# ha7ilm/csdr

Measured on AMD Instinct MI355X. Metric: complex MS/s in->out, WFM demod chain @2.4 MS/s x N streams, higher is better.
Workload: dtype f32

## Files before the change

### csdr_amd/csrc/wfm.hip

```cpp
#include "common.hpp"
#include "wfm_mfma.hpp"
#include "seeds.hpp"
#include <math.h>
#include <stdlib.h>
#include <vector>
#include <string>
#include <string.h>
using namespace csdr_amd;

namespace {

constexpr int HIST = WFM_HIST;
constexpr int TILE_A = 64;
constexpr int WARM = 48;

struct WfmParams {
    int D, L, F;
    int T;
    long long B;
    long long j_first;
    int n_audio;
};

__device__ __forceinline__ float u8_to_f(uint32_t v) { return fmaf((float)v, 0x1.010102p-7f, -1.0f); }
// ... 140 lines not shown
    size_t max_block;
    DevBuf<float> d_taps, d_demod, d_last[2];
    float phase;
    DevBuf<cf32> d_rot;
    DevBuf<uint8_t> d_hist;
    DevBuf<uint8_t> d_head[2]; int hflip;
    size_t demod_pitch;
    long long B, next_j;
    int last_T, flip;
    bool ended;
    std::string kernel_name;
    bool profiling;
    KernelTimer timer;
    double prof_ms; long prof_launches;
    bool use_mfma;
    WfmMfmaDevice mfma;
    DevBuf<> seq_frags; DevBuf<float> seq_cum; DevBuf<float2> dtab;
    DevBuf<float2> d_ctab; size_t ctab_cap;
    float2 c_prev;
    long long tab_first; bool tab_valid;
    bool ps; std::vector<float> rates, h_taps; DevBuf<float> d_scales;
    DevBuf<float2> d_dtab_old; DevBuf<int> d_lead_n; int *d_list; DevBuf<float> d_lead_d; std::vector<int> retuned;
    Owned<csdr_amd::SeedTables, seeds_destroy> seeds;
};

extern "C" {

static int wfm_upload_stream_tables(csdr_amd_wfm *w, int s, float rate)
{
    WfmMfmaTable t;
    wfm_mfma_build_table(w->D, w->L, w->F, rate, w->h_taps.data(), t);
    CSDR_HIP(hipMemcpy((uint8_t *)w->mfma.d_seq_frags + (size_t)s * t.seq_frags.size(), t.seq_frags.data(), t.seq_frags.size(), hipMemcpyHostToDevice));
    CSDR_HIP(hipMemcpy(w->mfma.d_seq_cum + (size_t)s * t.seq_cum.size(), t.seq_cum.data(), t.seq_cum.size() * sizeof(float), hipMemcpyHostToDevice));
    CSDR_HIP(hipMemcpy(w->mfma.d_dtab + (size_t)s * t.dtab.size(), t.dtab.data(), t.dtab.size() * sizeof(float2), hipMemcpyHostToDevice));
    CSDR_HIP(hipMemcpy(w->d_scales.get() + s, &t.seq_scale, sizeof(float), hipMemcpyHostToDevice));
    return 0;
}

static csdr_amd_wfm *wfm_create_impl(csdr_amd_ctx *ctx, int n_streams, const float *rates, bool per_stream, int decimation, const float *host_taps,
                                     int taps_length, int frac_rate, float tau, int audio_rate, size_t max_block_samples)
{
    const float shift_rate = rates ? rates[0] : 0.f;
    if (n_streams <= 0 || decimation <= 0 || taps_length <= 0 || frac_rate <= 1 || !rates) { fail_msg(-3, "wfm: bad parameters"); return nullptr; }
    if (decimation * 1 + taps_length + 8 > HIST) { fail_msg(-3, "wfm: D + taps (%d + %d) exceed the %d-sample history", decimation, taps_length, HIST); return nullptr; }
    if (max_block_samples < 1024) max_block_samples = 1024;
    Owned<csdr_amd_wfm, csdr_amd_wfm_destroy> w(new csdr_amd_wfm());
// ... 13 lines not shown
    alloc(w->d_taps, sizeof(float) * taps_length);
    alloc(w->d_last[0], sizeof(float) * n_streams);
    alloc(w->d_last[1], sizeof(float) * n_streams);
    if (w->use_mfma) {
        alloc(w->d_head[0], wfm_mfma_head_bytes(n_streams));
        alloc(w->d_head[1], wfm_mfma_head_bytes(n_streams));
    } else {
        alloc(w->d_demod, sizeof(float) * w->demod_pitch * n_streams);
        alloc(w->d_rot, sizeof(cf32) * (HIST + max_block_samples + 64));
        alloc(w->d_hist, (size_t)2 * HIST * n_streams);
    }
    if (e != hipSuccess) { fail(e, "hipMalloc(wfm state)", __FILE__, __LINE__); return nullptr; }
    (void)hipMemcpy(w->d_taps.get(), host_taps, sizeof(float) * taps_length, hipMemcpyHostToDevice);
    w->kernel_name = "k_wfm_front";
    if (w->use_mfma && per_stream) {
        WfmMfmaTable t;
        wfm_mfma_build_table(decimation, taps_length, frac_rate, shift_rate, host_taps, t);
        w->mfma.tile_stride_bytes = t.tile_stride_bytes; w->mfma.win_off_bytes = t.win_off_bytes; w->mfma.seq_scale = t.seq_scale;
        w->rates.assign(rates, rates + n_streams); w->h_taps.assign(host_taps, host_taps + taps_length);
        hipError_t e2 = dev_alloc(w->seq_frags, t.seq_frags.size() * (size_t)n_streams);
        if (e2 == hipSuccess) e2 = dev_alloc(w->seq_cum, t.seq_cum.size() * sizeof(float) * (size_t)n_streams);
        if (e2 == hipSuccess) e2 = dev_alloc(w->dtab, t.dtab.size() * sizeof(float2) * (size_t)n_streams);
        if (e2 == hipSuccess) e2 = dev_alloc(w->d_scales, sizeof(float) * (size_t)n_streams);
        w->mfma.d_seq_frags = w->seq_frags.get(); w->mfma.d_seq_cum = w->seq_cum.get(); w->mfma.d_dtab = w->dtab.get();
        if (e2 != hipSuccess) { fail(e2, "hipMalloc(wfm per-stream tables)", __FILE__, __LINE__); return nullptr; }
        for (int s = 0; s < n_streams; s++) if (wfm_upload_stream_tables(w.get(), s, rates[s])) return nullptr;
        w->seeds.reset(seeds_create(ctx, n_streams, rates, nullptr, 0, max_block_samples));
        if (!w->seeds) return nullptr;
        w->kernel_name = "k_wfm_mfma_seq";
    } else if (w->use_mfma) {
        WfmMfmaTable t;
        wfm_mfma_build_table(decimation, taps_length, frac_rate, shift_rate, host_taps, t);
        w->mfma.tile_stride_bytes = t.tile_stride_bytes; w->mfma.win_off_bytes = t.win_off_bytes; w->mfma.seq_scale = t.seq_scale;
        w->ctab_cap = 16 * (max_block_samples / 1024 + 8);
        hipError_t e2 = dev_alloc(w->d_ctab, w->ctab_cap * sizeof(float2));
        if (e2 == hipSuccess) e2 = dev_alloc(w->seq_frags, t.seq_frags.size());
        if (e2 == hipSuccess) e2 = dev_alloc(w->seq_cum, t.seq_cum.size() * sizeof(float));
        if (e2 == hipSuccess) e2 = dev_alloc(w->dtab, t.dtab.size() * sizeof(float2));
        w->mfma.d_seq_frags = w->seq_frags.get(); w->mfma.d_seq_cum = w->seq_cum.get(); w->mfma.d_dtab = w->dtab.get();
        if (e2 == hipSuccess) e2 = hipMemcpy(w->mfma.d_seq_frags, t.seq_frags.data(), t.seq_frags.size(), hipMemcpyHostToDevice);
        if (e2 == hipSuccess) e2 = hipMemcpy(w->mfma.d_seq_cum, t.seq_cum.data(), t.seq_cum.size() * sizeof(float), hipMemcpyHostToDevice);
        if (e2 == hipSuccess) e2 = hipMemcpy(w->mfma.d_dtab, t.dtab.data(), t.dtab.size() * sizeof(float2), hipMemcpyHostToDevice);
        if (e2 != hipSuccess) { fail(e2, "hipMalloc/hipMemcpy(wfm mfma table)", __FILE__, __LINE__); return nullptr; }
        w->kernel_name = "k_wfm_mfma_seq";
    }
    w->profiling = false; w->prof_ms = 0; w->prof_launches = 0;
// ... 126 lines not shown
    } else {
        if (w->last_T) CSDR_HIP(hipMemcpyAsync(w->d_rot.get(), w->d_rot.get() + w->last_T, sizeof(cf32) * HIST, hipMemcpyDeviceToDevice, st));
        rc = csdr_amd_rotator_generate(c, CSDR_SHIFT_ADDITION, w->shift_rate, &w->phase, w->d_rot.get() + HIST, (size_t)T, 1024, 0);
        if (rc) return rc;
    }
    const long long avail_last = w->B + T - 1;
    long long j_hi = -1;
    if (avail_last - (w->L - 1) >= 0) {
        const long long k_max = (avail_last - (w->L - 1)) / w->D;
        if (k_max >= 10) j_hi = (k_max - 10) / w->F;
    }
    const long long n_audio_ll = j_hi - w->next_j + 1;
    const int n_audio = n_audio_ll > 0 ? (int)n_audio_ll : 0;
    if (n_audio > 0 && (size_t)n_audio > out_pitch) return fail_msg(-3, "wfm: out_pitch %zu smaller than the %d audio samples of this block", out_pitch, n_audio);
    hipEvent_t e0 = nullptr, e1 = nullptr;
    if (w->profiling && n_audio > 0) { if (const int trc = w->timer.take(&e0, &e1)) return trc; }
    if (w->use_mfma) {
        WfmBackArgs back;
        back.alpha = w->alpha; back.last_in = w->d_last[w->flip].get(); back.last_out = w->d_last[w->flip ^ 1].get();
        back.s16 = audio_s16; back.af = audio_f; back.out_pitch = out_pitch; back.head_in = w->d_head[w->hflip].get(); back.head_out = w->d_head[w->hflip ^ 1].get();
        WfmPerStream psa; memset(&psa, 0, sizeof psa);
        if (w->ps) {
            psa.tab_pitch = sv.pitch; psa.tab_len = sv.n_entries; psa.d_scales = w->d_scales.get();
            long n_lead = 0; const int lead_max = wfm_lead_max(w->D, w->L, w->F);
            psa.lead_stride = lead_max;
            if (!w->retuned.empty() && n_audio > 0) {
                const long long lim = w->B - 1 - 9LL * w->D;
                if (lim >= 0) n_lead = (long)(lim / ((long long)w->D * w->F) - w->next_j + 1);
                if (n_lead < 0) n_lead = 0;
                if (n_lead > lead_max) n_lead = lead_max;
                if (n_lead > n_audio) n_lead = n_audio;
            }
            if (n_lead > 0) {
                const int nr = (int)w->retuned.size(), S = w->n_streams;
                if (!w->d_lead_n) { CSDR_HIP(dev_alloc(w->d_lead_n, sizeof(int) * 2 * S)); w->d_list = w->d_lead_n.get() + S; CSDR_HIP(dev_alloc(w->d_lead_d, sizeof(float) * (size_t)lead_max * S)); }
                int *hl = (int *)c->pinned_acquire(sizeof(int) * (size_t)(S + nr)); if (!hl) return -2;
                for (int s = 0; s < S; s++) hl[s] = 0;
                for (int k = 0; k < nr; k++) { hl[w->retuned[k]] = (int)n_lead; hl[S + k] = w->retuned[k]; }
                rc = c->pinned_upload(w->d_lead_n.get(), sizeof(int) * (size_t)(S + nr)); if (rc) return rc;
                rc = wfm_mfma_lead(st, in, in_pitch, back.head_in, w->d_taps.get(), sv.ctab, sv.pitch, w->mfma.d_dtab, w->d_dtab_old.get(), w->d_list, nr, w->d_lead_d.get(), lead_max,
                                   w->D, w->L, w->F, w->B, w->next_j, (int)n_lead);
                if (rc) return rc;
                psa.d_lead_d = w->d_lead_d.get(); psa.d_lead_n = w->d_lead_n.get();
            }
        }
        rc = wfm_mfma_launch(st, e0, e1, in, in_pitch, w->mfma, ctab_call, w->n_streams, T, w->B, w->next_j, n_audio, back, w->ps ? &psa : nullptr);
// ... 33 lines not shown
```

### csdr_amd/csrc/wfm_mfma.hip

```cpp
#include "common.hpp"
#include "wfm_mfma.hpp"
#include <hip/hip_ext.h>
#include <math.h>
#include <string.h>
#include <stdlib.h>
#include <complex>
#include <vector>
using namespace csdr_amd;

namespace csdr_amd {

bool wfm_mfma_supported(int D, int L, int F)
{
    if ((D * F) & 1) return false;
    const int win_off = (18 * D) & ~15;
    const int span_bytes = 2 * (D * (3 * F + 10) + L) - win_off;
    if (span_bytes > 64 * WFM_NK) return false;
    if (D + L + 3 * D * F + 8 > WFM_HIST) return false;
    return true;
}

void wfm_mfma_build_table(int D, int L, int F, float shift_rate, const float *taps, WfmMfmaTable &t)
{
    t.D = D; t.L = L; t.F = F;
// ... 89 lines not shown
#pragma unroll
            for (int l = 0; l < 3; l++) acc[l] = __builtin_amdgcn_mfma_i32_16x16x64_i8(A[ks * 3 + l], lo, acc[l], 0, 0, 0);
#pragma unroll
            for (int l = 0; l < 3; l++) snap[l] = acc[l];
#pragma unroll
            for (int l = 0; l < 3; l++) acc[l] = __builtin_amdgcn_mfma_i32_16x16x64_i8(A[ks * 3 + l], hi, acc[l], 0, 0, 0);
        } else {
#pragma unroll
            for (int l = 0; l < 3; l++) acc[l] = __builtin_amdgcn_mfma_i32_16x16x64_i8(A[ks * 3 + l], Bf[ks], acc[l], 0, 0, 0);
        }
    }
}

struct SeqParams {
    int n_streams; long long B2; long long tile_first; int n_tiles, tiles_per_seg;
    int stride, win_off; float scale;
    long long two_T;
    float alpha; const float *last_in; float *last_out; int16_t *s16; float *af; size_t out_pitch; long long j_first; int n_audio;
    const uint8_t *head_in; uint8_t *head_out;
    long long col_bytes; int col_chunks, col_audio, n_cols;
    size_t frag_stride, tab_pitch; int tab_len;
    const float *scales;
    const float *lead_d; const int *lead_n; int lead_stride;
};

#ifndef SEQ_RB_KIB
#define SEQ_RB_KIB 9
#endif
constexpr int SEQ_RB = 1024 * SEQ_RB_KIB;
#ifndef SEQ_RING_PAD
#define SEQ_RING_PAD 32
#endif
constexpr int SEQ_RP = SEQ_RB + SEQ_RING_PAD;
constexpr int SEQ_NGR = 4 * WFM_NK;
#ifndef SEQ_TPG_N
#define SEQ_TPG_N 6
#endif
#ifndef SEQ_NLD_N
#define SEQ_NLD_N 2
#endif
constexpr int SEQ_TPG = SEQ_TPG_N;
constexpr int SEQ_NLD = SEQ_NLD_N;
constexpr int SEQ_NW = SEQ_TPG + SEQ_NLD;
constexpr int SEQ_NLW = SEQ_NLD;
constexpr int SEQ_LINE = 64;
constexpr int SEQ_OUTS = (SEQ_LINE - 1 + 3 * 4 * SEQ_TPG + 4 * SEQ_TPG - 1) / (4 * SEQ_TPG);
// ... 14 lines not shown
#endif

constexpr int RES_WARM = 48;
struct ResCtl {
    const uint32_t *desc;
    const uint32_t *ctrl;
    uint32_t *done;
    unsigned *cnt;
    unsigned long long *t_first;
    unsigned long long *next_item;
    unsigned *exiting;
    const uint8_t *in_ring; int16_t *out_ring; size_t in_slot_bytes, out_slot_elems;
    int n_slots, desc_lines, n_wsb, T, D, L, F;
    long long idle_ticks, life_ticks;
    const float *lead_d; int lead_stride;
    const float *lead_state;
    unsigned long long *stats;
    int fence_mode;
};
__device__ __forceinline__ uint32_t sys_load(const uint32_t *p) { return __hip_atomic_load(p, __ATOMIC_RELAXED, __HIP_MEMORY_SCOPE_SYSTEM); }
__device__ __forceinline__ uint32_t res_tag(long long k) { return (uint32_t)((unsigned long long)k % 0xfffffffeull) + 1u; }

template <bool PS, bool RES = false>
__global__ __launch_bounds__(64 * SEQ_NW) void k_wfm_mfma_seq(const uint8_t *__restrict__ in, size_t in_pitch, const v4i *__restrict__ frags, const float *__restrict__ cum,
                                                               const float2 *__restrict__ dtab, const float2 *__restrict__ ctab, SeqParams p_in, ResCtl rc)
{
    static_assert(!(PS && RES), "the resident form exists for the shared-rate kernel");
    constexpr int TPG = SEQ_TPG, SPW = 16 / SEQ_NLW, NTHR = 64 * SEQ_NW;
    extern __shared__ float4 lds_raw[];
    uint8_t *lds_in = reinterpret_cast<uint8_t *>(lds_raw);
    float *lds_out = reinterpret_cast<float *>(lds_in + 16 * SEQ_RP);
    float *lcum = lds_out + 16 * SEQ_OUTP;
    float2 *ctl = reinterpret_cast<float2 *>(lcum + (SEQ_NGR + 1) * 16);
    const int tid = threadIdx.x, wv = __builtin_amdgcn_readfirstlane(tid >> 6), lane = tid & 63, col = lane & 15, q = lane >> 4;
    const bool fetches = wv >= TPG;
#ifdef WFM_PROF
    const long long t_entry = __builtin_readcyclecounter();
    long long t_first = t_entry, t_last = t_entry;
#endif
    const int fw = wv - TPG;
    float scale = p_in.scale;
    if constexpr (PS) { const int sbp = blockIdx.x; frags += (size_t)sbp * p_in.frag_stride; cum += (size_t)sbp * ((SEQ_NGR + 1) * 16); dtab += (size_t)sbp * 3072; ctab += sbp; scale = p_in.scales[sbp]; }
    for (int i = tid; i < (SEQ_NGR + 1) * 16; i += NTHR) lcum[i] = cum[i];
    v4i A[WFM_NK * 3];
#pragma unroll
    for (int s = 0; s < WFM_NK * 3; s++) A[s] = frags[s * 64 + lane];

    float c_lo[4], c_hi[4];
    {
        const float4 a = *reinterpret_cast<const float4 *>(cum + 4 * q), b = *reinterpret_cast<const float4 *>(cum + (size_t)SEQ_NGR * 16 + 4 * q);
        c_lo[0] = a.x; c_lo[1] = a.y; c_lo[2] = a.z; c_lo[3] = a.w; c_hi[0] = b.x; c_hi[1] = b.y; c_hi[2] = b.z; c_hi[3] = b.w;
    }
    const float K = 0.340447550238101026565118445432744920253753662109375f;
    SeqParams p_res;
    if constexpr (RES) p_res = p_in;
    const SeqParams &p = RES ? p_res : p_in;
    unsigned long long item = 0;
    long long res_t_launch = 0;
    uint32_t *const rctl = reinterpret_cast<uint32_t *>(ctl);
    const float2 *const lseed = ctl + 1;
    long long st_wait = 0, st_body = 0, st_done = 0, st_items = 0, st_t = 0;
    if constexpr (RES) { item = rc.next_item[blockIdx.x]; res_t_launch = wall_clock64(); st_t = res_t_launch; }
    bool pend = false; unsigned pend_c = 0; int pend_slot = 0, pend_n = 0; long long pend_k = 0;
    uint32_t pre_v[4] = {0u, 0u, 0u, 0u}; bool pre_valid = false;
    auto res_complete = [&]() {
        if constexpr (RES) {
            if (tid == 0 && pend) {
                pend = false;
                if (pend_c + 1 == (unsigned)rc.n_wsb) {
                    const unsigned long long tf = __hip_atomic_exchange(rc.t_first + pend_slot, ~0ull, __ATOMIC_RELAXED, __HIP_MEMORY_SCOPE_AGENT), td = (unsigned long long)wall_clock64();
                    __hip_atomic_store(rc.cnt + pend_slot, 0u, __ATOMIC_RELAXED, __HIP_MEMORY_SCOPE_AGENT);
                    uint32_t *dn = rc.done + (size_t)pend_slot * 16;
                    __hip_atomic_store(dn + 1, (uint32_t)pend_n, __ATOMIC_RELAXED, __HIP_MEMORY_SCOPE_SYSTEM);
                    __hip_atomic_store(dn + 2, (uint32_t)tf, __ATOMIC_RELAXED, __HIP_MEMORY_SCOPE_SYSTEM); __hip_atomic_store(dn + 3, (uint32_t)(tf >> 32), __ATOMIC_RELAXED, __HIP_MEMORY_SCOPE_SYSTEM);
                    __hip_atomic_store(dn + 4, (uint32_t)td, __ATOMIC_RELAXED, __HIP_MEMORY_SCOPE_SYSTEM); __hip_atomic_store(dn + 5, (uint32_t)(td >> 32), __ATOMIC_RELAXED, __HIP_MEMORY_SCOPE_SYSTEM);
                    asm volatile("s_waitcnt vmcnt(0)" ::: "memory");
                    __hip_atomic_store(dn, res_tag(pend_k), __ATOMIC_RELAXED, __HIP_MEMORY_SCOPE_SYSTEM);
                }
            }
        }
    };
    for (;;) {
    int res_slot = 0, res_lead = 0; long long res_k = 0; bool res_retuned = false;
    const uint8_t *pblock = nullptr;
    if constexpr (RES) {
        res_k = (long long)(item / (unsigned)rc.n_wsb);
        res_slot = (int)(res_k % rc.n_slots);
        if (wv == 0) {
            const uint32_t *dsc = rc.desc + (size_t)res_slot * rc.desc_lines * 16;
            const uint32_t tag = res_tag(res_k);
            const int nd = rc.desc_lines * 16;
            const long long t_wait = wall_clock64();
            uint32_t state = 0;
            for (int iter = 0;; iter++) {
                uint32_t v[4] = {0u, 0u, 0u, 0u};
                bool have = false;
                if (iter == 0 && pre_valid) {
#pragma unroll
                    for (int j = 0; j < 4; j++) v[j] = pre_v[j];
                    have = true;
                } else {
                    const uint32_t t0 = sys_load(dsc);
                    if (t0 == tag) {
#pragma unroll
                        for (int j = 0; j < 4; j++) { const int d = lane + 64 * j; v[j] = d < nd ? sys_load(dsc + d) : 0u; }
// ... 30 lines not shown
                __hip_atomic_store(rc.exiting, 1u, __ATOMIC_RELAXED, __HIP_MEMORY_SCOPE_AGENT); rc.next_item[blockIdx.x] = item;
                unsigned long long *sp = rc.stats + (size_t)blockIdx.x * 4;
                sp[0] += (unsigned long long)st_wait; sp[1] += (unsigned long long)st_body; sp[2] += (unsigned long long)st_done; sp[3] += (unsigned long long)st_items;
            }
            return;
        }
        if (tid == 0) { const long long t = wall_clock64(); st_wait += t - st_t; st_t = t; }
        res_lead = (int)(rctl[1] & 0xffu); res_retuned = (rctl[1] >> 8) & 1u;
        auto j_hi = [&](long long kk) -> long long {
            if (kk < 0) return -1;
            const long long avail_last = (kk + 1) * rc.T - 1;
            if (avail_last - (rc.L - 1) < 0) return -1;
            const long long k_max = (avail_last - (rc.L - 1)) / rc.D;
            return k_max >= 10 ? (k_max - 10) / rc.F : -1;
        };
        const long long jp = j_hi(res_k - 1), jn = j_hi(res_k);
        p_res.B2 = 2 * res_k * rc.T;
        p_res.j_first = jp + 1; p_res.n_audio = (int)(jn - jp);
        p_res.tile_first = p_res.j_first / 4; p_res.n_tiles = (int)((p_res.j_first + p_res.n_audio - 1) / 4 - p_res.tile_first + 1);
        p_res.tiles_per_seg = p_res.n_tiles;
        p_res.s16 = rc.out_ring + (size_t)res_slot * rc.out_slot_elems;
        if (tid == 0) (void)__hip_atomic_fetch_min(rc.t_first + res_slot, (unsigned long long)wall_clock64(), __ATOMIC_RELAXED, __HIP_MEMORY_SCOPE_AGENT);
    }
    const int sb = RES ? (int)(item % (unsigned)rc.n_wsb) : (int)blockIdx.x;
    const int seg_y = RES ? 0 : (int)blockIdx.y;
    const int col0 = PS ? 16 * seg_y : 0;
    if constexpr (RES) {
        in = rc.in_ring + (size_t)res_slot * rc.in_slot_bytes;
        pblock = rc.in_ring + (size_t)((res_slot + rc.n_slots - 1) % rc.n_slots) * rc.in_slot_bytes + (long long)sb * 16 * (long long)in_pitch;
    }
    const long long t0 = p.tile_first + (long long)seg_y * p.tiles_per_seg * (PS ? 16 : 1);
    long long t1 = t0 + p.tiles_per_seg; if (t1 > p.tile_first + p.n_tiles) t1 = p.tile_first + p.n_tiles;
    if (!RES && t0 >= t1) return;
    const int n_it = (int)(t1 - t0), n_grp = (n_it + TPG - 1) / TPG;
    const int n_lead = RES ? res_lead : ((PS && p.lead_n && seg_y == 0) ? p.lead_n[sb] : 0);
    const int n_warm = RES ? ((res_k > 0 && !res_retuned) ? 2 : 0) : ((PS || seg_y > 0) ? 2 : 0);
    const int last_stream = p.n_streams - 1;
    const int tstride = p.stride;
    const long long org = PS ? (long long)col0 * p.col_bytes : 0LL;
    long long wg = (t0 - (long long)n_warm * TPG) * tstride + p.win_off - p.B2 - org;
    const long long F0 = wg & ~1023LL;
    long long F_end = ((t1 - 1) * tstride + p.win_off - p.B2 - org + 64 * WFM_NK + 1023) & ~1023LL;
    { const long long row_end = ((p.two_T + 1023) & ~1023LL) - org; if (F_end > row_end) F_end = row_end; }
    long long F = F0;
    int fslot = (int)((F0 + 2 * SEQ_RB) % SEQ_RB), wslot = (int)((wg + 2 * SEQ_RB) % SEQ_RB);
    const uint32_t lds_in_addr = (uint32_t)(size_t)(__attribute__((address_space(3))) uint8_t *)lds_in;
    uint32_t voff[SPW], voff_h[SPW];
    long long row_lim[SPW];
#pragma unroll
    for (int r = 0; r < SPW; r++) {
        if constexpr (PS) {
            voff[r] = (uint32_t)((long long)(SPW * fw + r) * p.col_bytes) + 16u * lane;
            voff_h[r] = 16u * lane;
            row_lim[r] = p.two_T - (long long)(col0 + SPW * fw + r) * p.col_bytes;
        } else {
            const int srow = max(min(sb * 16 + SPW * fw + r, last_stream) - sb * 16, 0);
// ... 100 lines not shown
            auto entry = [&](long long wgs) {
                int ci = ps_base(wgs) + 1 + (lane >> 4) + (col0 + (lane & 15)) * p.col_chunks;
                ci = min(max(ci, 0), p.tab_len - 1);
                return ctab + (size_t)ci * p.tab_pitch;
            };
            const float2 *pa = entry(wg), *pb = entry(wg + step_b);
            asm volatile("global_load_dwordx2 %0, %2, off\n\tglobal_load_dwordx2 %1, %3, off" : "+v"(c0), "+v"(c1) : "v"(pa), "v"(pb) : "memory");
        }
        asm volatile("s_waitcnt vmcnt(0)" : "+v"(c0), "+v"(c1) :: "memory");
        if (ps_lane) {
            ctl[((-n_warm + 2) & 1) * 48 + lane] = make_float2(c0.x, c0.y);
            ctl[((-n_warm + 1 + 2) & 1) * 48 + lane] = make_float2(c1.x, c1.y);
        }
        ps_load(wg + 2 * step_b);
    }
    if (fetches) {
        while (F < F_end && F + 1024 <= wg + SEQ_RB) row_step();
        wait_for(wg + (long long)(TPG - 1) * tstride);
    }
    __syncthreads();
    const uint8_t *lrow = lds_in + col * SEQ_RP;
    const int s0 = sb * 16;
    float yst = 0.f;
    const float one_minus = 1 - p.alpha;
    const bool iir_wave = wv == 0, iir_lane = iir_wave && lane < 16;
    constexpr int QL = TPG, SPS = 4 * TPG;
    float bp[QL + 1];
    bp[0] = 1.f;
#pragma unroll
    for (int j = 1; j <= QL; j++) bp[j] = bp[j - 1] * one_minus;
    const float b2q = bp[QL] * bp[QL], b3q = b2q * bp[QL];
    float yst_first = 0.f;
    if (!RES && iir_wave && seg_y == 0) {
        yst = p.last_in[PS ? sb : min(s0 + col, last_stream)]; if (yst != yst) yst = 0.f;
        yst_first = yst;
    }
    if (RES && iir_wave && res_retuned) yst = rc.lead_state[min(s0 + col, last_stream)];
    const long long j_end = p.j_first + p.n_audio;
    const int seg_lo = (int)max(0LL, p.j_first - 4 * t0);
    const int seg_hi = (int)min(4LL * n_it, j_end - 4 * t0);
    const long long idx0 = 4 * t0 - p.j_first;
    auto col_lo = [&](int c) { return PS ? (col0 + c == 0 ? seg_lo : 0) : seg_lo; };
    auto col_hi = [&](int c) { return PS ? (int)max(0LL, min(4LL * n_it, j_end - 4 * (t0 + (long long)c * p.tiles_per_seg))) : seg_hi; };
    const bool emit_vec = ((((size_t)p.s16 | (size_t)p.af) & 15) == 0) && (p.out_pitch & 7) == 0;
    const int emit_a = (int)((SEQ_LINE - (idx0 & (SEQ_LINE - 1))) & (SEQ_LINE - 1));
    typedef unsigned wfm_st4 __attribute__((ext_vector_type(4)));
    auto put16 = [&](int16_t *dst, unsigned a, unsigned b, unsigned c, unsigned d) __attribute__((always_inline)) {
// ... 177 lines not shown
            const float dq = cQ - pQ, di = cI - pI;
            const float num = cI * dq - cQ * di, den = cI * cI + cQ * cQ;
            float rd = __builtin_amdgcn_rcpf(den);
            rd = fmaf(fmaf(-den, rd, 1.0f), rd, rd);
            float dval = (den != 0.f) ? (K * num) * rd : 0.f;
            if constexpr (PS) {
                const long long ja = 4 * (t0 + it) + q - p.j_first;
                if (n_lead > 0 && col0 + col == 0 && ja >= 0 && ja < n_lead) dval = p.lead_d[(size_t)sb * p.lead_stride + ja];
            }
            if constexpr (RES) {
                if (n_lead > 0) {
                    const long long ja = 4 * (t0 + it) + q - p.j_first;
                    if (ja >= 0 && ja < n_lead) dval = rc.lead_d[(size_t)min(sb * 16 + col, last_stream) * rc.lead_stride + ja];
                }
            }
            lout[col * SEQ_OUTP + 4 * wv + q] = dval;
        }
        PROF_T(0)
        const long long wg_n = wg + (long long)TPG * tstride;
        __syncthreads();
        PROF_T(2)
        if (!emit_vec) emit_scalar(gi - 1);
        if (ps_wave) { ps_store(gi + 2); ps_load(wg + 3LL * TPG * tstride); }
        PROF_T(4)
        if (iir_wave && WFM_DIAG < 5) {
            if (PS && gi == 0 && col0 + col == 0) yst = yst_first;
            const int lo = (gi == 0 && !(RES && n_warm)) ? col_lo(col) : 0;
            const int hi = gi < 0 ? SPS : max(0, min(SPS, col_hi(col) - gi * SPS));
            if (PS ? __all(lo == 0 && (hi & 3) == 0) : (lo == 0 && (hi & 3) == 0)) {
                float *row = lout + col * SEQ_OUTP + QL * q;
                const int nv = hi;
                float x[QL], z[QL], y[QL];
#pragma unroll
                for (int j = 0; j < QL; j += 2) {
                    const float2 v = *reinterpret_cast<const float2 *>(row + j);
                    const bool ok = QL * q + j < nv;
                    x[j] = ok ? v.x : 0.f; x[j + 1] = ok ? v.y : 0.f;
                }
                z[0] = p.alpha * x[0];
#pragma unroll
                for (int j = 1; j < QL; j++) z[j] = p.alpha * x[j] + one_minus * z[j - 1];
                const float ze_0 = __shfl(z[QL - 1], col, 64), ze_1 = __shfl(z[QL - 1], col + 16, 64), ze_2 = __shfl(z[QL - 1], col + 32, 64);
                float S = yst;
                if (q == 1) S = bp[QL] * yst + ze_0;
                else if (q == 2) S = b2q * yst + (bp[QL] * ze_0 + ze_1);
                else if (q == 3) S = b3q * yst + (b2q * ze_0 + (bp[QL] * ze_1 + ze_2));
#pragma unroll
                for (int j = 0; j < QL; j++) y[j] = z[j] + bp[j + 1] * S;
#pragma unroll
                for (int j = 0; j < QL; j += 2) *reinterpret_cast<float2 *>(row + j) = make_float2(y[j], y[j + 1]);
                if (nv > 0) {
                    const int lq = (nv - 1) / QL, lj = (nv - 1) % QL;
                    float ylast = y[QL - 1];
#pragma unroll
                    for (int j = 1; j < QL - 1; j += 2) if (lj == j) ylast = y[j];
                    yst = __shfl(ylast, col + 16 * lq, 64);
                }
            } else {
                float yv = yst;
                if (lane < 16) {
                    float *row = lout + col * SEQ_OUTP;
                    for (int i = lo; i < hi; i++) { yv = p.alpha * row[i] + one_minus * yv; row[i] = yv; }
                }
                yst = __shfl(yv, col, 64);
            }
        }
        PROF_T(5)
#ifdef WFM_PROF
        prof[6] += 1;
#endif
        wg = wg_n; wslot += TPG * tstride; if (wslot >= SEQ_RB) wslot -= SEQ_RB;
    }
#ifdef WFM_PROF
    if (lane == 0) for (int k = 0; k < 8; k++) atomicAdd(&g_wfm_prof[wv][k], (unsigned long long)prof[k]);
    t_last = __builtin_readcyclecounter();
#endif
    __syncthreads();
    if (!emit_vec) emit_scalar(n_grp - 1);
    }
    if (PS && seg_y + 1 == (int)gridDim.y) {
        if (iir_lane && col0 + lane == p.n_cols - 1) p.last_out[sb] = yst;
        if (tid < 32 && p.two_T >= 512 && (p.two_T & 15) == 0) {
            const uint4 v = *reinterpret_cast<const uint4 *>(in + (size_t)sb * in_pitch + (p.two_T - 512) + 16 * tid);
            *reinterpret_cast<uint4 *>(p.head_out + (size_t)sb * SEQ_HEAD + 512 + 16 * tid) = v;
        }
    } else
    if (!PS && !RES && seg_y + 1 == (int)gridDim.y) {
        if (iir_lane && s0 + lane < p.n_streams) p.last_out[s0 + lane] = yst;
        if (tid < 16 * 32 && p.two_T >= 512 && (p.two_T & 15) == 0 && s0 + tid / 32 < p.n_streams) {
            const int srow = tid / 32, piece = tid % 32;
            const uint4 v = *reinterpret_cast<const uint4 *>(sblock + (size_t)srow * in_pitch + (p.two_T - 512) + 16 * piece);
            *reinterpret_cast<uint4 *>(p.head_out + (size_t)(s0 + srow) * SEQ_HEAD + 512 + 16 * piece) = v;
        }
    }
#ifdef WFM_PROF
    if (lane == 0) {
        asm volatile("s_waitcnt vmcnt(0)" ::: "memory");
        const long long t_exit = __builtin_readcyclecounter();
        atomicAdd(&g_wfm_life[wv][0], (unsigned long long)(t_first - t_entry)); atomicAdd(&g_wfm_life[wv][1], (unsigned long long)(t_last - t_first));
        atomicAdd(&g_wfm_life[wv][2], (unsigned long long)(t_exit - t_last)); atomicAdd(&g_wfm_life[wv][3], 1ULL);
    }
#endif
    if constexpr (!RES) break;
    else {
        if (tid == 0) { const long long t = wall_clock64(); st_body += t - st_t; st_t = t; }
        if (wv == 0) {
            const unsigned long long nx = item + gridDim.x;
            const long long nk = (long long)(nx / (unsigned)rc.n_wsb);
            const uint32_t *dsc = rc.desc + (size_t)(nk % rc.n_slots) * rc.desc_lines * 16;
            const int nd = rc.desc_lines * 16;
#pragma unroll
            for (int j = 0; j < 4; j++) { const int d = lane + 64 * j; pre_v[j] = d < nd ? sys_load(dsc + d) : 0u; }
            pre_valid = true;
        }
        if (rc.fence_mode == 2) __threadfence_system();
        if (wv != 0 || !emit_vec) asm volatile("s_waitcnt vmcnt(0)" ::: "memory");
        __syncthreads();
        if (tid == 0) {
            if (rc.fence_mode == 3) __threadfence_system();
            pend_c = __hip_atomic_fetch_add(rc.cnt + res_slot, 1u, __ATOMIC_RELAXED, __HIP_MEMORY_SCOPE_AGENT);
            pend = true; pend_slot = res_slot; pend_n = p.n_audio; pend_k = res_k;
        }
        item += gridDim.x;
        if (tid == 0) { const long long t = wall_clock64(); st_done += t - st_t; st_t = t; st_items++; }
    }
    }
// ... 103 lines not shown
    const int n_wsb = (n_streams + 15) / 16;
    int n_seg = (n_cu + n_wsb - 1) / n_wsb; if (n_seg < 1) n_seg = 1;
    if (n_seg > sp.n_tiles / 24) n_seg = sp.n_tiles / 24;
    if (n_seg < 1) n_seg = 1;
    sp.tiles_per_seg = ((sp.n_tiles + n_seg - 1) / n_seg + SEQ_TPG - 1) / SEQ_TPG * SEQ_TPG;
    n_seg = (sp.n_tiles + sp.tiles_per_seg - 1) / sp.tiles_per_seg;
    sp.alpha = back.alpha; sp.last_in = back.last_in; sp.last_out = back.last_out; sp.s16 = back.s16; sp.af = back.af; sp.out_pitch = back.out_pitch;
    sp.j_first = j_first; sp.n_audio = n_audio; sp.head_in = back.head_in; sp.head_out = back.head_out;
    if (ps) {
        const long long ts = sp.stride / 2;
        long long per = ts; { long long a = per, b = 1024; while (b) { const long long t = a % b; a = b; b = t; } per = per / a * 1024; }
        int tpp = (int)(per / ts);
        while ((4 * tpp) % SEQ_LINE) tpp *= 2;
        const int n_per = (sp.n_tiles + tpp - 1) / tpp;
        int n_ss = (4 * n_cu + n_streams - 1) / n_streams; if (n_ss < 1) n_ss = 1;
        int np = (n_per + 16 * n_ss - 1) / (16 * n_ss); if (np < 1) np = 1;
        sp.tiles_per_seg = np * tpp;
        sp.n_cols = (sp.n_tiles + sp.tiles_per_seg - 1) / sp.tiles_per_seg;
        n_seg = (sp.n_cols + 15) / 16;
        sp.col_bytes = (long long)sp.tiles_per_seg * sp.stride; sp.col_chunks = (int)(sp.col_bytes / 2048); sp.col_audio = 4 * sp.tiles_per_seg;
        sp.frag_stride = (size_t)WFM_NK * 3 * 64; sp.tab_pitch = ps->tab_pitch; sp.tab_len = ps->tab_len; sp.scales = ps->d_scales;
        sp.lead_d = ps->d_lead_d; sp.lead_n = ps->d_lead_n; sp.lead_stride = ps->lead_stride;
        if (sp.col_bytes * 16 + 4096 >= (1LL << 32)) return fail_msg(-3, "wfm: block too large for the per-stream kernel's 32-bit row offsets");
        const size_t ldsp = (size_t)16 * SEQ_RP + 16 * SEQ_OUTP * sizeof(float) + (SEQ_NGR + 1) * 16 * sizeof(float) + 2 * 48 * sizeof(float2);
        { const int arc = lds_attr_once((const void *)k_wfm_mfma_seq<true>, ldsp); if (arc) return arc; }
        if (ev_begin && ev_end)
            hipExtLaunchKernelGGL(k_wfm_mfma_seq<true>, dim3(n_streams, n_seg), dim3(64 * SEQ_NW), ldsp, st, ev_begin, ev_end, 0, in, in_pitch, (const v4i *)dev.d_seq_frags, dev.d_seq_cum, dev.d_dtab, ctab, sp, no_res);
        else
            hipLaunchKernelGGL(k_wfm_mfma_seq<true>, dim3(n_streams, n_seg), dim3(64 * SEQ_NW), ldsp, st, in, in_pitch, (const v4i *)dev.d_seq_frags, dev.d_seq_cum, dev.d_dtab, ctab, sp, no_res);
        CSDR_LAUNCH_CHECK();
        if (T < 256 || (T & 7)) {
            hipLaunchKernelGGL(k_wfm_roll_head, dim3(n_streams), dim3(256), 0, st, in, in_pitch, 2LL * T, back.head_in, back.head_out);
            CSDR_LAUNCH_CHECK();
        }
        return 0;
    }
    const size_t lds = (size_t)16 * SEQ_RP + 16 * SEQ_OUTP * sizeof(float) + (SEQ_NGR + 1) * 16 * sizeof(float);
    { const int arc = lds_attr_once((const void *)k_wfm_mfma_seq<false>, lds); if (arc) return arc; }
    if (ev_begin && ev_end)
        hipExtLaunchKernelGGL(k_wfm_mfma_seq<false>, dim3(n_wsb, n_seg), dim3(64 * SEQ_NW), lds, st, ev_begin, ev_end, 0, in, in_pitch, (const v4i *)dev.d_seq_frags, dev.d_seq_cum, dev.d_dtab, ctab, sp, no_res);
    else
        hipLaunchKernelGGL(k_wfm_mfma_seq<false>, dim3(n_wsb, n_seg), dim3(64 * SEQ_NW), lds, st, in, in_pitch, (const v4i *)dev.d_seq_frags, dev.d_seq_cum, dev.d_dtab, ctab, sp, no_res);
    CSDR_LAUNCH_CHECK();
    if (T < 256 || (T & 7)) {
        hipLaunchKernelGGL(k_wfm_roll_head, dim3(n_streams), dim3(256), 0, st, in, in_pitch, 2LL * T, back.head_in, back.head_out);
        CSDR_LAUNCH_CHECK();
    }
    return 0;
}

int wfm_mfma_launch_resident(hipStream_t st, hipEvent_t ev_end, const WfmMfmaDevice &dev, int n_streams, size_t in_pitch, float alpha, size_t out_pitch, const WfmResident &rv, int grid)
{
// ... 83 lines not shown
```

### csdr_amd/csrc/wfm_mfma.hpp

```cpp
#pragma once
#include "common.hpp"
#include <vector>

namespace csdr_amd {

constexpr int WFM_HIST = 256;
constexpr int WFM_NK = 8;

struct WfmMfmaTable {
    int D, L, F, tile_stride_bytes, win_off_bytes;
    std::vector<int8_t> seq_frags;
    std::vector<float> seq_cum;
    std::vector<float2> dtab;
    float seq_scale;
};

struct WfmMfmaDevice {
    int tile_stride_bytes, win_off_bytes;
    void *d_seq_frags; float *d_seq_cum; float2 *d_dtab; float seq_scale;
};

struct WfmBackArgs {
    float alpha; const float *last_in; float *last_out; int16_t *s16; float *af; size_t out_pitch; const uint8_t *head_in; uint8_t *head_out;
};

struct WfmPerStream { size_t tab_pitch; int tab_len; const float *d_scales; const float *d_lead_d; const int *d_lead_n; int lead_stride; };
inline int wfm_lead_max(int D, int L, int F) { return (D + L - 1) / (D * F) + 2; }

struct WfmResident {
    const uint32_t *desc, *ctrl; uint32_t *done;
    unsigned *cnt; unsigned long long *t_first, *next_item; unsigned *exiting;
    const uint8_t *in_ring; int16_t *out_ring; size_t in_slot_bytes, out_slot_elems;
    int n_slots, desc_lines, T, D, L, F;
    long long idle_ticks, life_ticks;
    const float *lead_d, *lead_state; int lead_stride;
    unsigned long long *stats; int fence_mode;
};
constexpr int WFM_RES_WARM = 48;
int wfm_mfma_launch_resident(hipStream_t st, hipEvent_t ev_end, const WfmMfmaDevice &dev, int n_streams, size_t in_pitch, float alpha, size_t out_pitch, const WfmResident &rv, int grid);
int wfm_resident_max_grid();
int wfm_mfma_lead_shared(hipStream_t st, const uint8_t *in, size_t in_pitch, const uint8_t *prev, size_t two_T, const float *d_taps, const float2 *ctab, const float2 *d_dtab,
                         const float2 *d_dtab_old, const int *d_list, int n_list, float *d_lead_d, int lead_stride, float *d_warm, float *d_state, float alpha,
                         int D, int L, int F, long long B, long long j_first, int n_lead);

bool wfm_mfma_supported(int D, int L, int F);
void wfm_mfma_build_table(int D, int L, int F, float shift_rate, const float *taps, WfmMfmaTable &t);
size_t wfm_mfma_head_bytes(int n_streams);
int wfm_mfma_launch(hipStream_t st, hipEvent_t ev_begin, hipEvent_t ev_end, const uint8_t *in, size_t in_pitch, const WfmMfmaDevice &dev, const float2 *ctab,
                    int n_streams, int T, long long B, long long j_first, int n_audio, const WfmBackArgs &back, const WfmPerStream *ps = nullptr);
// ... 5 lines not shown
```

Measured before the change: 2.919 million.

## Run per-stream WFM kernel as persistent grid pulling work tickets atomically

The per-stream MFMA kernel can now launch a CU-sized persistent grid. Each block takes (stream, segment) tickets from a global atomic counter, reloads that stream's weights per ticket, and prefetches the next ticket near the end of the current one; the last block to finish resets the counter. This is meant to cut launch and tail overhead and balance uneven work across CUs. The cost is extra weight reloads per ticket, an additional barrier, and atomic traffic. It is enabled by default unless CSDR_AMD_WFM_WALK_GRID=0.

```diff
diff --git a/csdr_amd/csrc/wfm.hip b/csdr_amd/csrc/wfm.hip
--- a/csdr_amd/csrc/wfm.hip
+++ b/csdr_amd/csrc/wfm.hip
@@ -186,6 +186,7 @@
     bool ps; std::vector<float> rates, h_taps; DevBuf<float> d_scales;
     DevBuf<float2> d_dtab_old; DevBuf<int> d_lead_n; int *d_list; DevBuf<float> d_lead_d; std::vector<int> retuned;
     Owned<csdr_amd::SeedTables, seeds_destroy> seeds;
+    DevBuf<unsigned> d_walk; int walk_grid;
 };
 
 extern "C" {
@@ -245,6 +246,9 @@
         if (e2 == hipSuccess) e2 = dev_alloc(w->seq_cum, t.seq_cum.size() * sizeof(float) * (size_t)n_streams);
         if (e2 == hipSuccess) e2 = dev_alloc(w->dtab, t.dtab.size() * sizeof(float2) * (size_t)n_streams);
         if (e2 == hipSuccess) e2 = dev_alloc(w->d_scales, sizeof(float) * (size_t)n_streams);
+        if (e2 == hipSuccess) e2 = dev_alloc(w->d_walk, sizeof(unsigned) * 2);
+        if (e2 == hipSuccess) e2 = hipMemset(w->d_walk.get(), 0, sizeof(unsigned) * 2);
+        { const char *g = getenv("CSDR_AMD_WFM_WALK_GRID"); w->walk_grid = (g && *g) ? atoi(g) : -1; if (w->walk_grid < 0) w->walk_grid = -1; }
         w->mfma.d_seq_frags = w->seq_frags.get(); w->mfma.d_seq_cum = w->seq_cum.get(); w->mfma.d_dtab = w->dtab.get();
         if (e2 != hipSuccess) { fail(e2, "hipMalloc(wfm per-stream tables)", __FILE__, __LINE__); return nullptr; }
         for (int s = 0; s < n_streams; s++) if (wfm_upload_stream_tables(w.get(), s, rates[s])) return nullptr;
@@ -417,6 +421,7 @@
         WfmPerStream psa; memset(&psa, 0, sizeof psa);
         if (w->ps) {
             psa.tab_pitch = sv.pitch; psa.tab_len = sv.n_entries; psa.d_scales = w->d_scales.get();
+            psa.d_walk = w->d_walk.get(); psa.walk_grid = w->walk_grid;
             long n_lead = 0; const int lead_max = wfm_lead_max(w->D, w->L, w->F);
             psa.lead_stride = lead_max;
             if (!w->retuned.empty() && n_audio > 0) {
diff --git a/csdr_amd/csrc/wfm_mfma.hip b/csdr_amd/csrc/wfm_mfma.hip
--- a/csdr_amd/csrc/wfm_mfma.hip
+++ b/csdr_amd/csrc/wfm_mfma.hip
@@ -135,6 +135,7 @@
     size_t frag_stride, tab_pitch; int tab_len;
     const float *scales;
     const float *lead_d; const int *lead_n; int lead_stride;
+    int n_seg, n_tickets; unsigned *walk;
 };
 
 #ifndef SEQ_RB_KIB
@@ -195,8 +196,8 @@
 __device__ __forceinline__ uint32_t res_tag(long long k) { return (uint32_t)((unsigned long long)k % 0xfffffffeull) + 1u; }
 
 template <bool PS, bool RES = false>
-__global__ __launch_bounds__(64 * SEQ_NW) void k_wfm_mfma_seq(const uint8_t *__restrict__ in, size_t in_pitch, const v4i *__restrict__ frags, const float *__restrict__ cum,
-                                                               const float2 *__restrict__ dtab, const float2 *__restrict__ ctab, SeqParams p_in, ResCtl rc)
+__global__ __launch_bounds__(64 * SEQ_NW) void k_wfm_mfma_seq(const uint8_t *__restrict__ in, size_t in_pitch, const v4i *__restrict__ frags0, const float *__restrict__ cum0,
+                                                               const float2 *__restrict__ dtab0, const float2 *__restrict__ ctab0, SeqParams p_in, ResCtl rc)
 {
     static_assert(!(PS && RES), "the resident form exists for the shared-rate kernel");
     constexpr int TPG = SEQ_TPG, SPW = 16 / SEQ_NLW, NTHR = 64 * SEQ_NW;
@@ -205,25 +206,21 @@
     float *lds_out = reinterpret_cast<float *>(lds_in + 16 * SEQ_RP);
     float *lcum = lds_out + 16 * SEQ_OUTP;
     float2 *ctl = reinterpret_cast<float2 *>(lcum + (SEQ_NGR + 1) * 16);
-    const int tid = threadIdx.x, wv = __builtin_amdgcn_readfirstlane(tid >> 6), lane = tid & 63, col = lane & 15, q = lane >> 4;
-    const bool fetches = wv >= TPG;
-#ifdef WFM_PROF
-    const long long t_entry = __builtin_readcyclecounter();
+    const int tid = threadIdx.x, wv = __builtin_amdgcn_readfirstlane(tid >> 6), lane = tid & 63, q = lane >> 4;
+#ifdef WFM_PROF
+    long long t_entry = __builtin_readcyclecounter();
     long long t_first = t_entry, t_last = t_entry;
 #endif
-    const int fw = wv - TPG;
-    float scale = p_in.scale;
-    if constexpr (PS) { const int sbp = blockIdx.x; frags += (size_t)sbp * p_in.frag_stride; cum += (size_t)sbp * ((SEQ_NGR + 1) * 16); dtab += (size_t)sbp * 3072; ctab += sbp; scale = p_in.scales[sbp]; }
-    for (int i = tid; i < (SEQ_NGR + 1) * 16; i += NTHR) lcum[i] = cum[i];
     v4i A[WFM_NK * 3];
-#pragma unroll
-    for (int s = 0; s < WFM_NK * 3; s++) A[s] = frags[s * 64 + lane];
-
     float c_lo[4], c_hi[4];
-    {
+    auto load_weights = [&](const v4i *__restrict__ frags, const float *__restrict__ cum) __attribute__((always_inline)) {
+        for (int i = tid; i < (SEQ_NGR + 1) * 16; i += NTHR) lcum[i] = cum[i];
+#pragma unroll
+        for (int s = 0; s < WFM_NK * 3; s++) A[s] = frags[s * 64 + lane];
         const float4 a = *reinterpret_cast<const float4 *>(cum + 4 * q), b = *reinterpret_cast<const float4 *>(cum + (size_t)SEQ_NGR * 16 + 4 * q);
         c_lo[0] = a.x; c_lo[1] = a.y; c_lo[2] = a.z; c_lo[3] = a.w; c_hi[0] = b.x; c_hi[1] = b.y; c_hi[2] = b.z; c_hi[3] = b.w;
-    }
+    };
+    if constexpr (!PS) load_weights(frags0, cum0);
     const float K = 0.340447550238101026565118445432744920253753662109375f;
     SeqParams p_res;
     if constexpr (RES) p_res = p_in;
@@ -253,7 +250,32 @@
             }
         }
     };
+    const bool walking = PS && p_in.walk != nullptr;
+    unsigned *const tk_word = reinterpret_cast<unsigned *>(ctl + 2 * 48);
+    const bool tk_lane = walking && tid == 64;
+    unsigned tk_next = 0;
+    auto take_ticket = [&]() { return __hip_atomic_fetch_add(p_in.walk, 1u, __ATOMIC_RELAXED, __HIP_MEMORY_SCOPE_AGENT); };
+    if (tk_lane) tk_next = take_ticket();
     for (;;) {
+    int tk_sb = (int)blockIdx.x, tk_seg = (int)blockIdx.y;
+    if constexpr (PS) {
+        if (walking) {
+            if (tk_lane) *tk_word = tk_next;
+            __syncthreads();
+            const unsigned tk = (unsigned)__builtin_amdgcn_readfirstlane((int)*tk_word);
+            if (tk >= (unsigned)p_in.n_tickets) {
+                if (tk_lane && __hip_atomic_fetch_add(p_in.walk + 1, 1u, __ATOMIC_RELAXED, __HIP_MEMORY_SCOPE_AGENT) + 1 == gridDim.x) {
+                    __hip_atomic_store(p_in.walk, 0u, __ATOMIC_RELAXED, __HIP_MEMORY_SCOPE_AGENT);
+                    __hip_atomic_store(p_in.walk + 1, 0u, __ATOMIC_RELAXED, __HIP_MEMORY_SCOPE_AGENT);
+                }
+                return;
+            }
+            tk_sb = (int)(tk / (unsigned)p_in.n_seg); tk_seg = (int)(tk % (unsigned)p_in.n_seg);
+#ifdef WFM_PROF
+            t_entry = __builtin_readcyclecounter();
+#endif
+        }
+    }
     int res_slot = 0, res_lead = 0; long long res_k = 0; bool res_retuned = false;
     const uint8_t *pblock = nullptr;
     if constexpr (RES) {
@@ -330,8 +352,17 @@
         p_res.s16 = rc.out_ring + (size_t)res_slot * rc.out_slot_elems;
         if (tid == 0) (void)__hip_atomic_fetch_min(rc.t_first + res_slot, (unsigned long long)wall_clock64(), __ATOMIC_RELAXED, __HIP_MEMORY_SCOPE_AGENT);
     }
-    const int sb = RES ? (int)(item % (unsigned)rc.n_wsb) : (int)blockIdx.x;
-    const int seg_y = RES ? 0 : (int)blockIdx.y;
+    int tid_t = threadIdx.x; float alpha_t = p_in.alpha;
+    if constexpr (PS) asm volatile("" : "+v"(tid_t), "+s"(alpha_t));
+    const int tid = tid_t, wv = __builtin_amdgcn_readfirstlane(tid >> 6), lane = tid & 63, col = lane & 15, q = lane >> 4;
+    const bool fetches = wv >= TPG;
+    const int fw = wv - TPG;
+    const float alpha = alpha_t;
+    const int sb = RES ? (int)(item % (unsigned)rc.n_wsb) : tk_sb;
+    const int seg_y = RES ? 0 : tk_seg;
+    const float2 *const dtab = PS ? dtab0 + (size_t)sb * 3072 : dtab0, *const ctab = PS ? ctab0 + sb : ctab0;
+    const float scale = PS ? p_in.scales[sb] : p_in.scale;
+    if constexpr (PS) load_weights(frags0 + (size_t)sb * p_in.frag_stride, cum0 + (size_t)sb * ((SEQ_NGR + 1) * 16));
     const int col0 = PS ? 16 * seg_y : 0;
     if constexpr (RES) {
         in = rc.in_ring + (size_t)res_slot * rc.in_slot_bytes;
@@ -339,7 +370,7 @@
     }
     const long long t0 = p.tile_first + (long long)seg_y * p.tiles_per_seg * (PS ? 16 : 1);
     long long t1 = t0 + p.tiles_per_seg; if (t1 > p.tile_first + p.n_tiles) t1 = p.tile_first + p.n_tiles;
-    if (!RES && t0 >= t1) return;
+    if (!RES && t0 >= t1) { if (!walking) return; if (tk_lane) tk_next = take_ticket(); continue; }
     const int n_it = (int)(t1 - t0), n_grp = (n_it + TPG - 1) / TPG;
     const int n_lead = RES ? res_lead : ((PS && p.lead_n && seg_y == 0) ? p.lead_n[sb] : 0);
     const int n_warm = RES ? ((res_k > 0 && !res_retuned) ? 2 : 0) : ((PS || seg_y > 0) ? 2 : 0);
@@ -486,7 +517,7 @@
     const uint8_t *lrow = lds_in + col * SEQ_RP;
     const int s0 = sb * 16;
     float yst = 0.f;
-    const float one_minus = 1 - p.alpha;
+    const float one_minus = 1 - alpha;
     const bool iir_wave = wv == 0, iir_lane = iir_wave && lane < 16;
     constexpr int QL = TPG, SPS = 4 * TPG;
     float bp[QL + 1];
@@ -710,6 +741,7 @@
         PROF_T(2)
         if (!emit_vec) emit_scalar(gi - 1);
         if (ps_wave) { ps_store(gi + 2); ps_load(wg + 3LL * TPG * tstride); }
+        if (tk_lane && gi == n_grp - 2) tk_next = take_ticket();
         PROF_T(4)
         if (iir_wave && WFM_DIAG < 5) {
             if (PS && gi == 0 && col0 + col == 0) yst = yst_first;
@@ -725,9 +757,9 @@
                     const bool ok = QL * q + j < nv;
                     x[j] = ok ? v.x : 0.f; x[j + 1] = ok ? v.y : 0.f;
                 }
-                z[0] = p.alpha * x[0];
-#pragma unroll
-                for (int j = 1; j < QL; j++) z[j] = p.alpha * x[j] + one_minus * z[j - 1];
+                z[0] = alpha * x[0];
+#pragma unroll
+                for (int j = 1; j < QL; j++) z[j] = alpha * x[j] + one_minus * z[j - 1];
                 const float ze_0 = __shfl(z[QL - 1], col, 64), ze_1 = __shfl(z[QL - 1], col + 16, 64), ze_2 = __shfl(z[QL - 1], col + 32, 64);
                 float S = yst;
                 if (q == 1) S = bp[QL] * yst + ze_0;
@@ -748,7 +780,7 @@
                 float yv = yst;
                 if (lane < 16) {
                     float *row = lout + col * SEQ_OUTP;
-                    for (int i = lo; i < hi; i++) { yv = p.alpha * row[i] + one_minus * yv; row[i] = yv; }
+                    for (int i = lo; i < hi; i++) { yv = alpha * row[i] + one_minus * yv; row[i] = yv; }
                 }
                 yst = __shfl(yv, col, 64);
             }
@@ -765,8 +797,9 @@
 #endif
     __syncthreads();
     if (!emit_vec) emit_scalar(n_grp - 1);
-    }
-    if (PS && seg_y + 1 == (int)gridDim.y) {
+    if (ps_wave && walking) asm volatile("s_waitcnt vmcnt(0)" : "+v"(psC) :: "memory");
+    }
+    if (PS && seg_y + 1 == p.n_seg) {
         if (iir_lane && col0 + lane == p.n_cols - 1) p.last_out[sb] = yst;
         if (tid < 32 && p.two_T >= 512 && (p.two_T & 15) == 0) {
             const uint4 v = *reinterpret_cast<const uint4 *>(in + (size_t)sb * in_pitch + (p.two_T - 512) + 16 * tid);
@@ -789,7 +822,7 @@
         atomicAdd(&g_wfm_life[wv][2], (unsigned long long)(t_exit - t_last)); atomicAdd(&g_wfm_life[wv][3], 1ULL);
     }
 #endif
-    if constexpr (!RES) break;
+    if constexpr (!RES) { if (!walking) break; }
     else {
         if (tid == 0) { const long long t = wall_clock64(); st_body += t - st_t; st_t = t; }
         if (wv == 0) {
@@ -939,12 +972,19 @@
         sp.frag_stride = (size_t)WFM_NK * 3 * 64; sp.tab_pitch = ps->tab_pitch; sp.tab_len = ps->tab_len; sp.scales = ps->d_scales;
         sp.lead_d = ps->d_lead_d; sp.lead_n = ps->d_lead_n; sp.lead_stride = ps->lead_stride;
         if (sp.col_bytes * 16 + 4096 >= (1LL << 32)) return fail_msg(-3, "wfm: block too large for the per-stream kernel's 32-bit row offsets");
-        const size_t ldsp = (size_t)16 * SEQ_RP + 16 * SEQ_OUTP * sizeof(float) + (SEQ_NGR + 1) * 16 * sizeof(float) + 2 * 48 * sizeof(float2);
+        sp.n_seg = n_seg; sp.n_tickets = n_streams * n_seg;
+        dim3 grid(n_streams, n_seg);
+        if (ps->walk_grid != 0 && ps->d_walk) {
+            int g = n_cu < sp.n_tickets ? n_cu : sp.n_tickets;
+            if (ps->walk_grid > 0) g = ps->walk_grid < n_cu ? ps->walk_grid : n_cu;
+            grid = dim3(g); sp.walk = ps->d_walk;
+        }
+        const size_t ldsp = (size_t)16 * SEQ_RP + 16 * SEQ_OUTP * sizeof(float) + (SEQ_NGR + 1) * 16 * sizeof(float) + 2 * 48 * sizeof(float2) + 16;
         { const int arc = lds_attr_once((const void *)k_wfm_mfma_seq<true>, ldsp); if (arc) return arc; }
         if (ev_begin && ev_end)
-            hipExtLaunchKernelGGL(k_wfm_mfma_seq<true>, dim3(n_streams, n_seg), dim3(64 * SEQ_NW), ldsp, st, ev_begin, ev_end, 0, in, in_pitch, (const v4i *)dev.d_seq_frags, dev.d_seq_cum, dev.d_dtab, ctab, sp, no_res);
+            hipExtLaunchKernelGGL(k_wfm_mfma_seq<true>, grid, dim3(64 * SEQ_NW), ldsp, st, ev_begin, ev_end, 0, in, in_pitch, (const v4i *)dev.d_seq_frags, dev.d_seq_cum, dev.d_dtab, ctab, sp, no_res);
         else
-            hipLaunchKernelGGL(k_wfm_mfma_seq<true>, dim3(n_streams, n_seg), dim3(64 * SEQ_NW), ldsp, st, in, in_pitch, (const v4i *)dev.d_seq_frags, dev.d_seq_cum, dev.d_dtab, ctab, sp, no_res);
+            hipLaunchKernelGGL(k_wfm_mfma_seq<true>, grid, dim3(64 * SEQ_NW), ldsp, st, in, in_pitch, (const v4i *)dev.d_seq_frags, dev.d_seq_cum, dev.d_dtab, ctab, sp, no_res);
         CSDR_LAUNCH_CHECK();
         if (T < 256 || (T & 7)) {
             hipLaunchKernelGGL(k_wfm_roll_head, dim3(n_streams), dim3(256), 0, st, in, in_pitch, 2LL * T, back.head_in, back.head_out);
diff --git a/csdr_amd/csrc/wfm_mfma.hpp b/csdr_amd/csrc/wfm_mfma.hpp
--- a/csdr_amd/csrc/wfm_mfma.hpp
+++ b/csdr_amd/csrc/wfm_mfma.hpp
@@ -24,7 +24,7 @@
     float alpha; const float *last_in; float *last_out; int16_t *s16; float *af; size_t out_pitch; const uint8_t *head_in; uint8_t *head_out;
 };
 
-struct WfmPerStream { size_t tab_pitch; int tab_len; const float *d_scales; const float *d_lead_d; const int *d_lead_n; int lead_stride; };
+struct WfmPerStream { size_t tab_pitch; int tab_len; const float *d_scales; const float *d_lead_d; const int *d_lead_n; int lead_stride; unsigned *d_walk; int walk_grid; };
 inline int wfm_lead_max(int D, int L, int F) { return (D + L - 1) / (D * F) + 2; }
 
 struct WfmResident {
```

New measurement: 2.916 million. Within noise of the previous version (-0.1%).
